# markp-gc/ipu_path_trace

Measured on AMD Instinct MI355X. Metric: Mpath-samples/sec @1104x1000, 300 spp/step, depth 8, higher is better.
Workload: dtype f16

## Files before the change

ipu_path_trace_amd/csrc/pt_nif_group.h:

```cpp
#pragma once

#include "ptmi_share_plan.h"

namespace ptd {

constexpr unsigned long long kShareEmpty = ~0ull;
constexpr uint32_t kShareMaxProbes = 32;
constexpr int kShareBlock = 256;
constexpr uint32_t kClassInFlight = 2;
static_assert(kShareBlock == (int)ptshare::kClaimBlock, "the claim tiles of ptmi_share_plan.h are for this workgroup");

__device__ __forceinline__ uint32_t share_hash(unsigned long long k) {
  k ^= k >> 33; k *= 0xff51afd7ed558ccdull;
  k ^= k >> 33; k *= 0xc4ceb9fe1a85ec53ull;
  k ^= k >> 33;
  return (uint32_t)k;
}

__device__ __forceinline__ uint32_t lane_rank(uint64_t mask) {
  return __builtin_amdgcn_mbcnt_hi((uint32_t)(mask >> 32), __builtin_amdgcn_mbcnt_lo((uint32_t)mask, 0u));
}

__device__ __forceinline__ void wave_count(bool pred, unsigned long long* ctr) {
  const uint64_t m = __ballot(pred);
// ... 403 lines not shown
  uint32_t next = s_first + ptshare::claim_wave_offset(s_appends, wave);
#pragma unroll
  for (uint32_t k = 0; k < K; ++k) {
    const uint32_t bit = 1u << k;
    const size_t q = q0 + ptshare::claim_entry(tile, threadIdx.x, k);
    const uint64_t m = __ballot((append & bit) != 0);
    if (append & bit) {
      const uint32_t i = next + lane_rank(m);
      M.c_u[i] = u[k]; M.c_v[i] = v[k];
      const uint32_t g = M.c_base + i;
      if (fresh & bit) __hip_atomic_store(M.words + slot[k], g, __ATOMIC_RELAXED, __HIP_MEMORY_SCOPE_AGENT);
      Q.owner[q] = g;
    } else if (valid & bit) {
      Q.owner[q] = ptshare::owner_is_store(word[k]) ? word[k] : ptshare::owner_class(slot[k]);
    }
    next += (uint32_t)__popcll(m);
  }
}

__global__ __launch_bounds__(kShareBlock) void class_map_claim_kernel(GroupQueue Q, ClassMap M) { class_map_claim(Q, M); }
__global__ __launch_bounds__(kShareBlock) void class_map_expand_kernel(GroupExpand E, ClassMap M) { group_expand(E, M); }
__global__ __launch_bounds__(kShareBlock) void share_raw_claim_kernel(GroupQueue Q, RawCountTable T) { group_claim(Q, T); }

__global__ __launch_bounds__(kShareBlock) void class_map_release_kernel(const float* c_u, const float* c_v, const uint32_t* c_count,
                                                                        uint32_t region, uint32_t* words) {
  const uint32_t n = c_count[blockIdx.y];
  const size_t base = (size_t)blockIdx.y * region;
  for (uint32_t i = blockIdx.x * (uint32_t)kShareBlock + threadIdx.x; i < n; i += gridDim.x * (uint32_t)kShareBlock) {
    const uint32_t slot = ptshare::class_map_index(c_u[base + i], c_v[base + i]);
    if (slot != ptshare::kClassIrregular) words[slot] = ptshare::kMapEmpty;
  }
}

__global__ __launch_bounds__(kShareBlock) void class_claim_kernel(GroupQueue Q, ClassTable T) { group_claim(Q, T); }
__global__ __launch_bounds__(kShareBlock) void class_resolve_kernel(GroupQueue Q, ClassTable T) { group_resolve(Q, T); }

__global__ __launch_bounds__(kShareBlock) void class_spread_kernel(const uint32_t* count, const uint32_t* owner, const float* class_bgr,
                                                                   float* bgr) {
  const uint32_t n = *count;
  for (uint32_t i = blockIdx.x * (uint32_t)kShareBlock + threadIdx.x; i < n; i += gridDim.x * (uint32_t)kShareBlock) {
    const float* from = class_bgr + 3 * (size_t)owner[i];
    const float b = from[0], g = from[1], r = from[2];
    float* to = bgr + 3 * (size_t)i;
    to[0] = b; to[1] = g; to[2] = r;
  }
}

}
```

ipu_path_trace_amd/csrc/pt_trace.h:

```cpp
#pragma once
#include "pt_device_math.h"
#include "pt_env_guide.h"
#include "pt_mesh.h"
#include "ptmi_trace_variant.h"

#include <utility>

namespace ptd {

enum { MAT_DIFFUSE = 0, MAT_SPECULAR = 1, MAT_REFRACTIVE = 2, MAT_EMISSIVE = 3 };
constexpr int kMaxObjects = 32;
constexpr int kBuiltinObjects = 6;
constexpr float kEps = 1e-5f;
constexpr float kInf = 3.402823466e+38f;
constexpr float kPi = 3.1415927410125732421875f;

struct SceneObject {
  float cx, cy, cz;
  float radius, r2;
  float nx, ny, nz;
  float colr, colg, colb;
  int32_t type;
  int32_t is_disc;
  float ocx, ocy, ocz;
  float c4;
  float kdisc;
  int32_t same_centre;
// ... 24 lines not shown
constexpr int kHitObjectBits = 5;
static_assert((1 << kHitObjectBits) == kMaxObjects, "5 bits of object in a packed hit");

struct TraceParams {
  SceneObject obj[kMaxObjects];
  uint32_t n_objects;
  float width_f, height_f;
  uint32_t width, height;
  float tx, ty;
  float aa_scale;
  float stop_prob;
  float rr_factor;
  float ri;
  float azimuth;
  uint32_t seed_lo, seed_hi;
  uint32_t sample_base;
  uint32_t max_path_length, roulette_depth;
  int32_t aa_type, samples_half;
  uint32_t n_items, total_paths;
  uint32_t n_waves;
  uint32_t region_cap;
  int32_t env_const;
  float env_r, env_g, env_b;
  const uint32_t* pix;
  float* q_u; float* q_v; float* q_tr; float* q_tg; float* q_tb; uint32_t* q_path;
  uint32_t* region_count;
  uint8_t* plen;
  float* rad_r; float* rad_g; float* rad_b;
  uint4* survivors;
  float4* states;
  size_t state_stride;
  uint32_t div_magic, div_shift;
  unsigned long long* diag;
  unsigned long long* emitted;
  int32_t cam_pose;
  float cam_r[3], cam_u[3], cam_f[3];
  float lens_a, lens_f;
  GuideParams guide;
  LightParams lights;
  PolyEdges poly[kMaxObjects];
  const ptmesh::Node* mesh_nodes;
  const ptmesh::F4* mesh_tris;
  const uint32_t* mesh_orig;
  const ptmesh::F4* mesh_normals;
};
static_assert(sizeof(TraceParams) <= 4096, "the scene travels in the kernel arguments: 4 KiB at most");
// ... 557 lines not shown
  if (s.depth >= P.max_path_length) {
    length = s.depth;
    return STEP_DEAD;
  }
  return STEP_CONTINUE;
}

__device__ __forceinline__ void dir_to_uv(Vec3 d, float azimuth, float& u, float& v) {
  float theta = dm_acos(d.y);
  float phi = dm_atan2(d.z, d.x) + azimuth;
  const float twoPi = 2.f * kPi;
  const float invPi = 1.f / kPi;
  const float inv2Pi = 1.f / twoPi;
  if (phi < 0.f) phi += twoPi;
  else if (phi > twoPi) phi -= twoPi;
  u = theta * invPi;
  v = phi * inv2Pi;
}

constexpr int kTraceBlock = 256;
constexpr uint32_t kRefillThreshold = 16;

__device__ __forceinline__ uint32_t emit_emitted(const TraceParams& P, bool emitted, Vec3 rad, uint32_t idx) {
  if (emitted) { P.rad_r[idx] = rad.x; P.rad_g[idx] = rad.y; P.rad_b[idx] = rad.z; }
  return (uint32_t)__popcll(__ballot(emitted));
}

template <int CAM = CAM_BUILTIN>
__device__ __forceinline__ void emit_escaped(const TraceParams& P, bool escaped, const PathState& st, uint32_t idx, uint32_t lane,
                                             uint32_t region_base, uint32_t* wg_count) {
  if (P.env_const) {
    if (escaped) {
      P.rad_r[idx] = P.env_r * st.T.x;
      P.rad_g[idx] = P.env_g * st.T.y;
      P.rad_b[idx] = P.env_b * st.T.z;
    }
    return;
  }
  const uint64_t esc_mask = __ballot(escaped);
  if (!esc_mask) return;
  uint32_t base = 0;
  if (lane == (uint32_t)__ffsll((long long)esc_mask) - 1u) base = atomicAdd(wg_count, (uint32_t)__popcll(esc_mask));
  base = __shfl(base, __ffsll((long long)esc_mask) - 1, 64);
  if (escaped) {
    const uint32_t rank = __builtin_amdgcn_mbcnt_hi((uint32_t)(esc_mask >> 32), __builtin_amdgcn_mbcnt_lo((uint32_t)esc_mask, 0u));
    const uint32_t q = region_base + base + rank;
    float u, v;
    Vec3 d = st.d;
    if constexpr (CAM != CAM_BUILTIN) { if (CAM == CAM_POSE || P.cam_pose) d = to_world(P, d); }
    dir_to_uv(d, P.azimuth, u, v);
    P.q_u[q] = u; P.q_v[q] = v;
    P.q_tr[q] = st.T.x; P.q_tg[q] = st.T.y; P.q_tb[q] = st.T.z;
    P.q_path[q] = idx;
  }
}

__device__ __forceinline__ uint32_t pack_half2(float a, float b) {
  union { _Float16 h[2]; uint32_t u; } c;
  c.h[0] = (_Float16)a; c.h[1] = (_Float16)b;
  return c.u;
}

#ifdef PTMI_DIAG_BUILD
}
#include "diag/pt_trace_r3fn.h"
#include "diag/pt_trace_rounds.h"
namespace ptd {
#endif

constexpr int kTraceOpt = 3;
template <uint32_t REFILL, int OPT = kTraceOpt, int CAM = CAM_BUILTIN, bool GUIDE = false, bool LIGHTS = false, bool POLY = false,
          bool PLAMPS = false, bool MESH = false, bool SMOOTH = false, bool TEX = false>
__device__ __forceinline__ void trace_body(const TraceParams& P, [[maybe_unused]] const TexParams* X = nullptr) {
  constexpr bool MAGIC = (OPT & 1) != 0, PRIMARY = (OPT & 2) != 0, SCENE_C = (OPT & 128) != 0, PIPE = (OPT & 256) != 0;
  __shared__ uint32_t wg_count;
  __shared__ uint32_t wg_front, wg_back;
// ... 332 lines not shown
```

ipu_path_trace_amd/csrc/ptmi.hip:

```cpp
#include <hip/hip_runtime.h>
#include <rccl/rccl.h>

#include <dlfcn.h>
#include <limits.h>

#include <algorithm>
#include <array>
#include <atomic>
#include <chrono>
#include <cmath>
#include <cfloat>
#include <cstdio>
#include <cstdlib>
#include <condition_variable>
#include <cstring>
#include <deque>
#include <functional>
#include <memory>
#include <mutex>
#include <string>
#include <thread>
#include <utility>
#include <vector>

// ... 513 lines not shown
        if (h->env_const) return PT_OK;
        ptd::NifParams N = h->nif;
        if (mode.classes)
          bind_dense_queue(N, h->group.d_class_u + b.class_base, h->group.d_class_v + b.class_base, h->group.d_class_count + b.index,
                           b.store_cap, h->group.d_class_bgr + 3 * (size_t)b.class_base);
        else if (mode.grouped()) bind_store_queue(h, N, b.index, b.store_base, b.store_cap);
        else bind_path_queue(N, B, b.g.blocks, b.g.region_cap);
#ifdef PTMI_DIAG_BUILD
        if (h->diag_fault_batch >= 0 && (uint32_t)h->diag_fault_batch == b.index)
          return fail(h, PT_ERR_HIP, "injected fault: NIF launch of batch " + std::to_string(b.index));
#endif
        if (int rc = h->env_map ? launch_envmap(h, N) : launch_nif(h, N, h->n_cus)) return rc;
        B.last_paths = b.total; B.last_regions = b.g.blocks; B.last_region_cap = b.g.region_cap;
        B.share_batch = mode.grouped() ? (int32_t)b.index : -1; B.share_base = b.store_base; B.share_region_cap = b.store_cap;
        h->stats.nif_launches += 1;
        return PT_OK;
      }, &done)) return rc;
  if (mode.classes && !mode.fused())
    if (int rc = stage_class_spread(h, ev, b, &done)) return rc;
  PT_HIP(hipStreamWaitEvent(h->acc_stream, done, 0));
  return PT_OK;
}

static int stage_accumulate(pt_handle h, StepEvents& ev, const Batch& b) {
  const pt_context::BatchBuffers& B = *b.B;
  const uint32_t n = h->n_items;
  if (int rc = ev.timed(h->acc_stream, pt_context::kSpanAccumulate, [&]() -> int {
        if (n % 4u == 0)
          hipLaunchKernelGGL(ptd::accumulate4_kernel, dim3((n / 4u + 255) / 256), dim3(256), 0, h->acc_stream, n, b.iters, B.plen,
                             B.rad_r, B.rad_g, B.rad_b, h->acc, h->d_counters);
        else
          hipLaunchKernelGGL(ptd::accumulate_kernel, dim3((n + 255) / 256), dim3(256), 0, h->acc_stream, n, b.iters, B.plen, B.rad_r,
                             B.rad_g, B.rad_b, h->acc, h->d_counters);
        PT_HIP(hipGetLastError());
        return PT_OK;
      })) return rc;
  PT_HIP(hipEventRecord(B.accumulated, h->acc_stream));
  h->stats.trace_launches += 1;
  h->stats.accumulate_launches += 1;
  return PT_OK;
}

static int enqueue_path_trace(pt_handle h) {
  const uint32_t n = h->n_items;
  if (int rc = ensure_meshes(h)) return rc;
  forget_replay_state(h);
  PT_HIP(hipMemsetAsync(h->d_counters, 0, 4 * sizeof(unsigned long long), h->stream));
  ptd::TraceParams P;
  fill_trace_params(h, P);
  P.n_items = n;
  StepEvents ev{h};
  hipEvent_t e_begin = nullptr, e_acc = nullptr, e_end = nullptr, e_class_cleared = nullptr;
  size_t e_acc_i = 0;
  if (int rc = ev.record(h->stream, e_begin, h->e_begin_i)) return rc;
  PT_HIP(hipStreamWaitEvent(h->trace_stream, e_begin, 0));
  const std::vector<uint32_t> deal = ptplan::batch_iterations(h->samples_per_step, h->iters_per_batch, h->first_batch_iters, h->env_const);
  const uint32_t batches = (uint32_t)deal.size();
  const int32_t share = h->group.share_mode_set ? h->group.share_mode : auto_share_mode(h, batches);
  StepMode mode{h->env_const ? 0 : share, !h->env_const && h->group.memo_slots != 0};
  h->group.share_mode_last = mode.share;
  h->group.memo_ran = mode.memo;
  if (mode.grouped()) {
    if (int rc = prepare_group_store(h, mode, batches)) return rc;
    if (int rc = prepare_class_level(h, ev, batches, mode, e_class_cleared)) return rc;
  }
  h->group.class_ran = mode.classes;
  if (mode.memo)
    if (int rc = ev.timed(h->trace_stream, pt_context::kSpanMemo, [&]() { return enqueue_memo_prologue(h); })) return rc;

  const bool handoff = mode.kind() == ptshare::StepKind::kStep;
  hipEvent_t e_clean = nullptr;
  uint32_t store_cap = 0, first_iter = 0;
  for (uint32_t i = 0; i < batches; first_iter += deal[i], ++i) {
    const uint32_t slot = ptplan::ring_slot(i, h->ring_depth);
    Batch b{i, first_iter, deal[i], deal[i] * n, trace_grid(deal[i] * n, h->trace_blocks), &h->bb[slot], 0u, 0u, slot};
    b.store_base = mode.grouped() ? ptplan::store_region(i, h->ring_depth, mode.step_scope()) * (uint32_t)h->queue_cap : 0u;
    b.store_cap = b.g.blocks * b.g.region_cap;
    b.class_base = mode.classes ? i * (uint32_t)h->queue_cap : 0u;
    store_cap = std::max(store_cap, b.store_cap);
    if (mode.mapped && ptplan::ring_predecessor(i, h->ring_depth) != ptplan::kNoBatch)
      PT_HIP(hipStreamWaitEvent(h->trace_stream, b.B->raw_read, 0));
    if (int rc = stage_trace(h, ev, P, b)) return rc;
    if (mode.grouped())
      if (int rc = stage_group(h, ev, mode, b, e_class_cleared)) return rc;
    if (int rc = stage_nif(h, ev, mode, b)) return rc;
    if (handoff && i + 1 == batches && !mode.mapped)
      if (int rc = enqueue_table_handoff(h, ev, e_clean, h->trace_stream)) return rc;
    if (mode.grouped())
      if (int rc = stage_expand(h, ev, mode, b)) return rc;
    if (int rc = stage_accumulate(h, ev, b)) return rc;
    if (mode.mapped)
      if (int rc = stage_raw_pairs(h, ev, b)) return rc;
    if (handoff && i + 1 == batches && mode.mapped)
      if (int rc = enqueue_table_handoff(h, ev, e_clean, h->acc_stream)) return rc;
  }
  if (e_clean) PT_HIP(hipStreamWaitEvent(h->stream, e_clean, 0));

  if (mode.mapped)
    if (int rc = stage_map_release(h, ev, store_cap, batches)) return rc;
  if (int rc = ev.record(h->acc_stream, e_acc, e_acc_i)) return rc;
  PT_HIP(hipStreamWaitEvent(h->stream, e_acc, 0));
  if (mode.memo)
    if (int rc = stage_memo_publish(h, ev, store_cap, batches)) return rc;
  PT_HIP(hipMemcpyAsync(h->h_counters, h->d_counters, 4 * sizeof(unsigned long long), hipMemcpyDeviceToHost, h->stream));
  if (mode.grouped()) {
    PT_HIP(hipMemcpyAsync(h->group.h_share_count, h->group.d_share_count, (size_t)batches * 4, hipMemcpyDeviceToHost, h->stream));
    PT_HIP(hipMemcpyAsync(h->group.h_share_over, h->group.d_share_over, 8, hipMemcpyDeviceToHost, h->stream));
  }
  if (mode.classes) {
    PT_HIP(hipMemcpyAsync(h->group.h_class_count, h->group.d_class_count, (size_t)batches * 4, hipMemcpyDeviceToHost, h->stream));
    PT_HIP(hipMemcpyAsync(h->group.h_class_over, h->group.d_class_over, 8, hipMemcpyDeviceToHost, h->stream));
  }
  if (mode.memo) PT_HIP(hipMemcpyAsync(h->group.h_memo_ctr, h->group.d_memo_ctr, ptd::kMemoCounters * 8, hipMemcpyDeviceToHost, h->stream));
// ... 13 lines not shown
    else if (s.kind == pt_context::kSpanShare) h->group.share_ms += ms;
    else if (s.kind == pt_context::kSpanClass) h->group.class_ms += ms;
    else h->group.memo_ms += ms;
  }
  float total_ms = 0.f;
  PT_HIP(hipEventElapsedTime(&total_ms, h->events[h->e_begin_i], h->events[h->e_end_i]));
  h->stats.total_ms = total_ms;
  return PT_OK;
}

extern "C" {

int pt_path_trace(pt_handle h) {
  if (!h) return PT_ERR_INVALID_ARGUMENT;
  if (!h->settings_valid) return fail(h, PT_ERR_NOT_READY, "pt_set_render_settings has not been called");
  if (!h->env_const && !h->env_map && !h->nif_valid)
    return fail(h, PT_ERR_NOT_READY, "no environment: call pt_upload_nif, pt_set_env_map or pt_set_constant_env");
  PT_HIP(hipSetDevice(h->cfg.device));
  memset(&h->stats, 0, sizeof(h->stats));
  h->group.share_mode_last = 0; h->group.share_evals = 0; h->group.share_overflowed = 0; h->group.share_ms = 0;
  h->group.memo_ran = false; h->group.memo_served = 0; h->group.memo_inserted = 0; h->group.memo_ms = 0;
  h->group.class_ran = false; h->group.class_rows = 0; h->group.class_alone = 0; h->group.class_ms = 0;
  h->group.class_map_ran = false;
  h->spans_pending = false;
  h->stats.nif_flops_per_sample = (h->env_const || h->env_map) ? 0 : h->nif_flops;
  h->stats.first_sample = h->sample_cursor;
  const uint32_t n = h->n_items;
  if (n == 0) return PT_OK;

  h->spans.clear();
  const int rc = enqueue_path_trace(h);
  hipError_t s0 = hipStreamSynchronize(h->stream), s1 = hipSuccess, s2 = hipSuccess, s3 = hipSuccess;
  if (rc || s0 != hipSuccess) {
    for (hipStream_t cs : h->chunk_stream) { const hipError_t e = hipStreamSynchronize(cs); if (e != hipSuccess) s3 = e; }
    s1 = hipStreamSynchronize(h->trace_stream);
    s2 = hipStreamSynchronize(h->acc_stream);
    (void)hipStreamSynchronize(h->stream);
  }
  const bool failed = rc || s0 != hipSuccess || s1 != hipSuccess || s2 != hipSuccess || s3 != hipSuccess;
  if (failed) memo_new_generation(h);
  h->group.share_clean_slots = ptshare::mark_after_step(h->group.share_clean_slots,
      StepMode{h->group.share_mode_last, h->group.memo_ran}.kind(), h->group.share_slots, !failed);
  h->group.class_map_clean = ptshare::map_mark_after_step(h->group.class_map_clean, h->group.class_map_ran, !failed);
  if (rc) return rc;
  for (hipError_t e : {s0, s1, s2, s3})
    if (e != hipSuccess) return fail(h, PT_ERR_HIP, std::string("path_trace: ") + hipGetErrorString(e));
// ... 752 lines not shown
```

ipu_path_trace_amd/csrc/ptmi_context.h:

```cpp
#pragma once

using ptplan::TraceGrid;
using ptplan::trace_grid;
using ptplan::item_divider;

namespace {

thread_local std::string g_create_error;

inline uint32_t f2u(float f) { uint32_t u; memcpy(&u, &f, 4); return u; }
inline float u2f(uint32_t u) { float f; memcpy(&f, &u, 4); return f; }

uint16_t host_f2h(float f) {
  uint32_t x = f2u(f), sign = (x >> 16) & 0x8000u, ax = x & 0x7fffffffu;
  if (ax >= 0x7f800000u) return (uint16_t)(sign | 0x7c00u | ((ax > 0x7f800000u) ? 0x200u : 0u));
  if (ax >= 0x477ff000u) return (uint16_t)(sign | 0x7c00u);
  if (ax < 0x33000001u) return (uint16_t)sign;
  int e = (int)(ax >> 23) - 127;
  uint32_t m = (ax & 0x7fffffu) | 0x800000u, shift, hexp;
  if (e < -14) { shift = (uint32_t)(13 + (-14 - e)); hexp = 0; } else { shift = 13; hexp = (uint32_t)(e + 15); }
  uint32_t q = m >> shift, rem = m & ((1u << shift) - 1u), halfway = 1u << (shift - 1);
  if (rem > halfway || (rem == halfway && (q & 1u))) q += 1u;
  uint32_t h = hexp == 0 ? q : ((hexp - 1u) << 10) + q;
  return (uint16_t)(sign | h);
// ... 285 lines not shown

    DevBuf<unsigned long long> d_class_keys;
    DevBuf<uint32_t> d_class_vals;
    uint32_t class_slots = 0;
    uint32_t class_diag_slots = 0;
    DevBuf<uint32_t> d_class_owner;
    DevBuf<float> d_class_u, d_class_v, d_class_bgr;
    size_t class_regions = 0;
    DevBuf<uint32_t> d_class_count;
    DevBuf<unsigned long long> d_class_over;
    PinnedBuf<uint32_t> h_class_count;
    PinnedBuf<unsigned long long> h_class_over;
    size_t class_count_cap = 0;
    bool class_failed = false;
    bool class_ran = false;
    uint64_t class_rows = 0, class_alone = 0;
    double class_ms = 0;
    DevBuf<uint32_t> d_class_map;
    DevBuf<unsigned long long> d_class_tail_keys;
    uint32_t class_tail_slots = 0;
    bool class_map_clean = false;
    bool class_map_failed = false;
    bool class_map_ran = false;

    DevBuf<ptd::MemoSlot> d_memo;
    uint32_t memo_slots = 0;
    DevBuf<ptd::MemoSlot> d_memo_list;
    DevBuf<uint32_t> d_memo_slot;
    size_t memo_slot_regions = 0;
    DevBuf<unsigned long long> d_memo_ctr;
    PinnedBuf<unsigned long long> h_memo_ctr;
    bool memo_clear = false;
    uint32_t memo_step = 0;
    bool memo_ran = false;
    uint64_t memo_occupied = 0, memo_served = 0, memo_inserted = 0, memo_generation = 0, memo_retains = 0;
    double memo_ms = 0;
  } group;

  pt_stats stats{};
  std::vector<hipEvent_t> events;
  enum SpanKind { kSpanNone = -1, kSpanTrace, kSpanNif, kSpanAccumulate, kSpanShare, kSpanMemo, kSpanClass };
  struct StageSpan { size_t a, b; int kind; };
  std::vector<StageSpan> spans;
  size_t e_begin_i = 0, e_end_i = 0;
  bool spans_pending = false;

// ... 308 lines not shown
```

ipu_path_trace_amd/csrc/ptmi_nif_group.h:

```cpp
#pragma once

static int resolve_stage_times(pt_handle h);


static uint64_t free_device_bytes() {
  size_t free_b = 0, total_b = 0;
  return hipMemGetInfo(&free_b, &total_b) == hipSuccess ? (uint64_t)free_b : ptshare::kFreeUnknown;
}

static uint32_t share_table_slots(pt_handle h, uint64_t entries, uint64_t free_b) {
  if (h->group.share_diag_slots) return h->group.share_diag_slots;
  return ptshare::worst_case_slots(entries, free_b);
}

static int ensure_share_counts(pt_handle h, size_t batches) {
  if (batches <= h->group.share_count_cap) return PT_OK;
  h->group.share_count_cap = 0;
  PT_HIP(dev_alloc(h->group.d_share_count, batches));
  PT_HIP(dev_alloc(h->group.h_share_count, batches));
  h->group.share_count_cap = batches;
  return PT_OK;
}

static int ensure_share_store(pt_handle h, size_t regions) {
// ... 113 lines not shown
  } else if (2 * h->group.memo_occupied > h->group.memo_slots) {
    const uint32_t list_cap = std::max<uint32_t>(1, h->group.memo_slots / 2);
    const uint32_t grid = std::min<uint32_t>(ptd::kMemoGrid, (h->group.memo_slots + ptd::kShareBlock - 1) / ptd::kShareBlock);
    hipLaunchKernelGGL(ptd::memo_compact_kernel, dim3(grid), dim3(ptd::kShareBlock), 0, s, h->group.d_memo, h->group.memo_slots, last,
                       h->group.d_memo_list, list_cap, h->group.d_memo_ctr);
    PT_HIP(hipGetLastError());
    PT_HIP(hipMemsetAsync(h->group.d_memo, 0xff, table_bytes, s));
    PT_HIP(hipMemsetAsync(h->group.d_memo_ctr + ptd::kMemoOccupied, 0, 8, s));
    const uint32_t rgrid = std::min<uint32_t>(ptd::kMemoGrid, (list_cap + ptd::kShareBlock - 1) / ptd::kShareBlock);
    hipLaunchKernelGGL(ptd::memo_reinsert_kernel, dim3(rgrid), dim3(ptd::kShareBlock), 0, s, h->group.d_memo, h->group.memo_slots - 1u,
                       h->group.d_memo_list, list_cap, h->group.d_memo_ctr);
    PT_HIP(hipGetLastError());
    h->group.memo_retains += 1;
  }
  return PT_OK;
}

struct StepMode {
  int32_t share;
  bool memo;
  bool classes = false;
  bool fused() const { return classes && !memo && share == PT_NIF_SHARE_STEP; }
  bool mapped = false;
  bool grouped() const { return share || memo; }
  bool step_scope() const { return memo || share == PT_NIF_SHARE_STEP; }
  ptshare::StepKind kind() const {
    return memo ? ptshare::StepKind::kMemo : share == PT_NIF_SHARE_STEP ? ptshare::StepKind::kStep
           : share == PT_NIF_SHARE_BATCH ? ptshare::StepKind::kBatch : ptshare::StepKind::kOff;
  }
};

static int32_t auto_share_mode(pt_handle h, size_t batches) {
  if (h->env_const || h->env_map || h->group.memo_slots || h->group.share_auto_failed) return PT_NIF_SHARE_OFF;
  const uint64_t free_b = free_device_bytes();
  const uint64_t slots = share_table_slots(h, batches * (uint64_t)h->queue_cap, free_b);
  ptshare::Held held;
  held.table_slots = h->group.d_share_keys ? (h->group.share_diag_slots ? slots : h->group.share_slots) : 0;
  held.store_regions = h->group.share_regions;
  for (const auto& o : h->group.d_share_owner) held.owner_maps += o ? 1 : 0;
  if (!ptshare::auto_fits(slots, batches, h->queue_cap, held, free_b, pt_context::kBatchSets)) return PT_NIF_SHARE_OFF;
  if (ensure_group_buffers(h, false, true, batches) == PT_OK && alloc_group_buffers(h) == PT_OK) return PT_NIF_SHARE_STEP;
  (void)hipGetLastError();
  free_share_buffers(h);
  h->group.share_auto_failed = true;
  h->error.clear();
  return PT_NIF_SHARE_OFF;
// ... 214 lines not shown
          else hipLaunchKernelGGL(ptd::share_claim_kernel, tiles, block, 0, h->trace_stream, Q, share_table(h));
        }
        PT_HIP(hipGetLastError());
        return PT_OK;
      })) return rc;
  return resolve_on_nif_stream(mode) ? PT_OK : stage_resolve(h, ev, mode, b, h->trace_stream);
}

static int stage_expand(pt_handle h, StepEvents& ev, const StepMode& mode, const Batch& b) {
  return ev.timed(h->acc_stream, mode.memo ? pt_context::kSpanMemo : pt_context::kSpanShare, [&]() -> int {
    const pt_context::BatchBuffers& B = *b.B;
    ptd::GroupExpand X;
    X.region_count = B.region_count;
    X.region_cap = b.g.region_cap;
    X.owner = h->group.d_share_owner[b.set()];
    X.bgr = mode.fused() ? h->group.d_class_bgr : h->group.d_share_bgr;
    X.q_tr = B.q_tr; X.q_tg = B.q_tg; X.q_tb = B.q_tb; X.q_path = B.q_path;
    X.rad_r = B.rad_r; X.rad_g = B.rad_g; X.rad_b = B.rad_b;
    if (mode.memo) hipLaunchKernelGGL(ptd::memo_expand_kernel, b.group_grid(), dim3(ptd::kShareBlock), 0, h->acc_stream, X, memo_table(h));
    else if (mode.mapped) hipLaunchKernelGGL(ptd::class_map_expand_kernel, b.group_grid(), dim3(ptd::kShareBlock), 0, h->acc_stream, X, class_map(h, b));
    else if (mode.fused()) hipLaunchKernelGGL(ptd::share_class_expand_kernel, b.group_grid(), dim3(ptd::kShareBlock), 0, h->acc_stream, X, share_class_table(h, b));
    else hipLaunchKernelGGL(ptd::share_expand_kernel, b.group_grid(), dim3(ptd::kShareBlock), 0, h->acc_stream, X, share_table(h));
    PT_HIP(hipGetLastError());
    return PT_OK;
  });
}

static int stage_raw_pairs(pt_handle h, StepEvents& ev, const Batch& b) {
  if (int rc = ev.timed(h->acc_stream, pt_context::kSpanShare, [&]() -> int {
        hipLaunchKernelGGL(ptd::share_raw_claim_kernel, b.claim_grid(), dim3(ptd::kShareBlock), 0, h->acc_stream, group_queue(h, b),
                           ptd::RawCountTable{share_table(h)});
        PT_HIP(hipGetLastError());
        return PT_OK;
      })) return rc;
  PT_HIP(hipEventRecord(b.B->raw_read, h->acc_stream));
  return PT_OK;
}

static int stage_map_release(pt_handle h, StepEvents& ev, uint32_t store_cap, uint32_t batches) {
  return ev.timed(h->acc_stream, pt_context::kSpanShare, [&]() -> int {
    const dim3 grid(std::min<uint32_t>(ptd::kMemoGrid, (store_cap + ptd::kShareBlock - 1u) / ptd::kShareBlock), batches);
    hipLaunchKernelGGL(ptd::class_map_release_kernel, grid, dim3(ptd::kShareBlock), 0, h->acc_stream, h->group.d_class_u, h->group.d_class_v,
                       h->group.d_class_count, (uint32_t)h->queue_cap, h->group.d_class_map);
    PT_HIP(hipGetLastError());
    PT_HIP(hipMemsetAsync(h->group.d_class_map + ptshare::kClassMapWords, 0xff, (size_t)h->group.class_tail_slots * 4, h->acc_stream));
    PT_HIP(hipMemsetAsync(h->group.d_class_tail_keys, 0xff, (size_t)h->group.class_tail_slots * 8, h->acc_stream));
    return PT_OK;
  });
}

static int stage_memo_publish(pt_handle h, StepEvents& ev, uint32_t store_cap, uint32_t batches) {
  return ev.timed(h->stream, pt_context::kSpanMemo, [&]() -> int {
    const dim3 grid(std::min<uint32_t>(ptd::kMemoGrid, (store_cap + ptd::kShareBlock - 1u) / ptd::kShareBlock), batches);
    hipLaunchKernelGGL(ptd::memo_publish_kernel, grid, dim3(ptd::kShareBlock), 0, h->stream, h->group.d_memo, h->group.d_memo_slot,
                       h->group.d_share_bgr, h->group.d_share_count, (uint32_t)h->queue_cap, h->group.memo_step);
    PT_HIP(hipGetLastError());
    return PT_OK;
  });
}

extern "C" {

int pt_set_nif_sharing(pt_handle h, int32_t mode) {
  if (!h) return PT_ERR_INVALID_ARGUMENT;
  if (mode != PT_NIF_SHARE_OFF && mode != PT_NIF_SHARE_BATCH && mode != PT_NIF_SHARE_STEP)
    return fail(h, PT_ERR_INVALID_ARGUMENT, "pt_set_nif_sharing: mode must be PT_NIF_SHARE_OFF, _BATCH or _STEP");
  if (mode != PT_NIF_SHARE_OFF) {
    PT_HIP(hipSetDevice(h->cfg.device));
    if (int rc = alloc_share_buffers(h)) { h->group.share_mode = PT_NIF_SHARE_OFF; h->group.share_mode_set = true; return rc; }
// ... 158 lines not shown
  PT_HIP(hipMemcpyAsync(owner, own, n * 4, hipMemcpyDeviceToHost, s));
  PT_HIP(hipMemcpyAsync(d_u, du, n * 4, hipMemcpyDeviceToHost, s));
  PT_HIP(hipMemcpyAsync(d_v, dv, n * 4, hipMemcpyDeviceToHost, s));
  PT_HIP(hipMemcpyAsync(d_count, len, 4, hipMemcpyDeviceToHost, s));
  PT_HIP(hipMemcpyAsync(overflowed, over, 8, hipMemcpyDeviceToHost, s));
  if (memo == 1 && memo_counters) PT_HIP(hipMemcpyAsync(memo_counters, ctr, ptd::kMemoCounters * 8, hipMemcpyDeviceToHost, s));
  if (table_keys) {
    if (memo == 1) PT_HIP(hipMemcpy2DAsync(table_keys, 8, slots, sizeof(ptd::MemoSlot), 8, table_slots, hipMemcpyDeviceToHost, s));
    else PT_HIP(hipMemcpyAsync(table_keys, keys, (size_t)table_slots * 8, hipMemcpyDeviceToHost, s));
  }
  PT_HIP(hipStreamSynchronize(s));
  return PT_OK;
}

int pt_diag_set_nif_class_capacity(pt_handle h, uint32_t slots) {
  if (!h || slots > ptshare::kClassMaxSlots) return PT_ERR_INVALID_ARGUMENT;
  uint32_t p = slots ? 2 : 0;
  while (p < slots) p <<= 1;
  h->group.class_diag_slots = p;
  h->group.class_failed = false;
  return PT_OK;
}

int pt_diag_class_claim(pt_handle h, const float* u, const float* v, uint32_t n, uint32_t table_slots, uint32_t* owner, float* c_u,
                        float* c_v, uint32_t* c_count, uint64_t* alone) {
  if (!h || !u || !v || !owner || !c_u || !c_v || !c_count || !alone) return PT_ERR_INVALID_ARGUMENT;
  if (n == 0 || n >= ptshare::kMaxStoreEntries || table_slots < 2 || table_slots > ptshare::kClassMaxSlots || (table_slots & (table_slots - 1u)))
    return fail(h, PT_ERR_INVALID_ARGUMENT, "pt_diag_class_claim: sizes out of range");
  PT_HIP(hipSetDevice(h->cfg.device));
  hipStream_t s = h->stream;
  DevBuf<float> q_u, q_v, du, dv;
  DevBuf<uint32_t> count, own, len, vals;
  DevBuf<unsigned long long> over, keys;
  PT_HIP(dev_alloc(q_u, n)); PT_HIP(dev_alloc(q_v, n)); PT_HIP(dev_alloc(du, n)); PT_HIP(dev_alloc(dv, n));
  PT_HIP(dev_alloc(count, 1)); PT_HIP(dev_alloc(own, n)); PT_HIP(dev_alloc(len, 1)); PT_HIP(dev_alloc(over, 1));
  PT_HIP(dev_alloc(keys, table_slots)); PT_HIP(dev_alloc(vals, table_slots));
  PT_HIP(hipMemcpyAsync(q_u, u, (size_t)n * 4, hipMemcpyHostToDevice, s));
  PT_HIP(hipMemcpyAsync(q_v, v, (size_t)n * 4, hipMemcpyHostToDevice, s));
  PT_HIP(hipMemcpyAsync(count, &n, 4, hipMemcpyHostToDevice, s));
  PT_HIP(hipMemsetAsync(own, 0xff, (size_t)n * 4, s));
  PT_HIP(hipMemsetAsync(over, 0, 8, s));
  PT_HIP(hipMemsetAsync(len, 0, 4, s));
  PT_HIP(hipMemsetAsync(keys, 0xff, (size_t)table_slots * 8, s));
  ptd::GroupQueue Q;
  Q.q_u = q_u; Q.q_v = q_v; Q.region_count = count; Q.region_cap = n; Q.owner = own;
  Q.d_u = du; Q.d_v = dv; Q.d_count = len; Q.base = 0; Q.overflowed = over;
// ... 100 lines not shown
  PT_HIP(hipSetDevice(h->cfg.device));
  hipStream_t s = h->stream;
  DevBuf<float> q_u, q_v, cu, cv;
  DevBuf<uint32_t> counts, own, row, len, words;
  DevBuf<unsigned long long> over, tail_keys;
  PT_HIP(dev_alloc(q_u, n)); PT_HIP(dev_alloc(q_v, n)); PT_HIP(dev_alloc(cu, 2 * n)); PT_HIP(dev_alloc(cv, 2 * n));
  PT_HIP(dev_alloc(counts, n_regions)); PT_HIP(dev_alloc(own, n)); PT_HIP(dev_alloc(row, n)); PT_HIP(dev_alloc(len, 1)); PT_HIP(dev_alloc(over, 3));
  PT_HIP(dev_alloc(words, n_words)); PT_HIP(dev_alloc(tail_keys, tail_slots));
  PT_HIP(hipMemcpyAsync(q_u, u, n * 4, hipMemcpyHostToDevice, s));
  PT_HIP(hipMemcpyAsync(q_v, v, n * 4, hipMemcpyHostToDevice, s));
  PT_HIP(hipMemcpyAsync(counts, region_count, (size_t)n_regions * 4, hipMemcpyHostToDevice, s));
  PT_HIP(hipMemsetAsync(over, 0, 24, s));
  PT_HIP(hipMemsetAsync(len, 0, 4, s));
  PT_HIP(hipMemsetAsync(words, 0xff, n_words * 4, s));
  PT_HIP(hipMemsetAsync(tail_keys, 0xff, (size_t)tail_slots * 8, s));
  ptd::GroupQueue Q;
  Q.q_u = q_u; Q.q_v = q_v; Q.region_count = counts; Q.region_cap = region_cap; Q.owner = own;
  Q.d_u = nullptr; Q.d_v = nullptr; Q.d_count = nullptr; Q.base = 0; Q.overflowed = nullptr;
  const ptd::ClassMap M{words, tail_keys, tail_slots - 1u, cu, cv, len, 0u, over};
  const dim3 grid((region_cap + ptd::kShareBlock - 1u) / ptd::kShareBlock, n_regions), tiles(ptshare::claim_tiles(region_cap), n_regions);
  const dim3 block(ptd::kShareBlock), count_grid(ptd::kMemoGrid);
  auto release = [&]() -> int {
    hipLaunchKernelGGL(ptd::class_map_release_kernel, dim3(std::min<uint32_t>(ptd::kMemoGrid, (uint32_t)((2 * n + ptd::kShareBlock - 1u) / ptd::kShareBlock)), 1),
                       block, 0, s, cu, cv, len, 0u, words);
    PT_HIP(hipGetLastError());
    PT_HIP(hipMemsetAsync(words + ptshare::kClassMapWords, 0xff, (size_t)tail_slots * 4, s));
    PT_HIP(hipMemsetAsync(tail_keys, 0xff, (size_t)tail_slots * 8, s));
    return PT_OK;
  };
  for (uint32_t launch = 0; launch < launches; ++launch) {
    if (launch && release_between) {
      if (int rc = release()) return rc;
      PT_HIP(hipMemsetAsync(len, 0, 4, s));
      PT_HIP(hipMemsetAsync(over, 0, 8, s));
    }
    PT_HIP(hipMemsetAsync(own, 0xff, n * 4, s));
    hipLaunchKernelGGL(ptd::class_map_claim_kernel, tiles, block, 0, s, Q, M);
    PT_HIP(hipGetLastError());
  }
  hipLaunchKernelGGL(ptd::diag_map_hop_kernel, grid, block, 0, s, counts, region_cap, own, words, row);
  PT_HIP(hipGetLastError());
  hipLaunchKernelGGL(ptd::diag_map_count_kernel, count_grid, block, 0, s, words, (uint32_t)n_words, over + 1);
  PT_HIP(hipGetLastError());
  if (int rc = release()) return rc;
  hipLaunchKernelGGL(ptd::diag_map_count_kernel, count_grid, block, 0, s, words, (uint32_t)n_words, over + 2);
  PT_HIP(hipGetLastError());
  uint32_t h_len = 0;
  unsigned long long h_over[3] = {0, 0, 0};
  PT_HIP(hipMemcpyAsync(owner, own, n * 4, hipMemcpyDeviceToHost, s));
  PT_HIP(hipMemcpyAsync(rows, row, n * 4, hipMemcpyDeviceToHost, s));
// ... 13 lines not shown
```

ipu_path_trace_amd/csrc/ptmi_share_plan.h:

```cpp
#pragma once

#include <cstdint>

namespace ptshare {

constexpr uint32_t kOwnerTagged = 0x80000000u;
constexpr uint32_t kOwnerPending = 0xc0000000u;
constexpr uint32_t kOwnerSlotBits = 0x3fffffffu;
constexpr uint32_t owner_served(uint32_t slot) { return kOwnerTagged | slot; }
constexpr uint32_t owner_pending(uint32_t slot) { return kOwnerPending | slot; }
constexpr bool owner_is_store(uint32_t o) { return !(o & kOwnerTagged); }
constexpr bool owner_is_pending(uint32_t o) { return (o & kOwnerPending) == kOwnerPending; }
constexpr bool owner_is_served(uint32_t o) { return (o & kOwnerPending) == kOwnerTagged; }
constexpr uint32_t owner_slot(uint32_t o) { return o & kOwnerSlotBits; }

constexpr uint32_t owner_class(uint32_t class_slot) { return kOwnerTagged | class_slot; }
constexpr bool owner_is_class(uint32_t o) { return (o & kOwnerPending) == kOwnerTagged; }
constexpr uint32_t kNoWriteBack = ~0u;
template <class RawVals, class ClassVals>
constexpr uint32_t resolve_two_hops(uint32_t o, const RawVals& raw_vals, const ClassVals& class_vals, uint32_t* write_back = nullptr) {
  if (write_back) *write_back = kNoWriteBack;
  if (owner_is_pending(o)) {
    const uint32_t s = owner_slot(o);
    o = raw_vals[s];
// ... 85 lines not shown
}
constexpr uint32_t class_coord(float coord) { return class_x((coord - 1.0f) * 2.0f); }
constexpr uint64_t class_key(float u, float v) { return ((uint64_t)class_coord(u) << 32) | (uint64_t)class_coord(v); }

constexpr uint32_t kClassAxis = ((kClassMaxMag - kClassMinMag) >> 13) + 1u;
constexpr uint32_t kClassMapWords = kClassAxis * kClassAxis;
constexpr uint32_t kClassIrregular = ~0u;
constexpr uint32_t kClassTailSlots = 1u << 16;
constexpr uint32_t kClassTailMaxSlots = 1u << 20;
static_assert((uint64_t)kClassMapWords + kClassTailMaxSlots - 1 <= kOwnerSlotBits, "a class slot fits an owner word");
constexpr uint32_t kMapEmpty = 0xffffffffu;
constexpr uint32_t kMapClaimed = 0xfffffffeu;
constexpr uint32_t class_axis_index(uint32_t c) {
  const uint32_t mag = c & 0x7fffffffu;
  return (c >> 31) && !(c & 0x1fffu) && mag >= kClassMinMag && mag <= kClassMaxMag ? (mag - kClassMinMag) >> 13 : kClassIrregular;
}
constexpr uint32_t class_map_index(float u, float v) {
  const uint32_t iu = class_axis_index(class_coord(u)), iv = class_axis_index(class_coord(v));
  return iu == kClassIrregular || iv == kClassIrregular ? kClassIrregular : iu * kClassAxis + iv;
}
constexpr uint64_t class_map_bytes(uint32_t tail_slots) { return ((uint64_t)kClassMapWords + tail_slots) * 4 + (uint64_t)tail_slots * 8; }
constexpr bool map_clear_skippable(bool mark) { return mark; }
constexpr bool map_mark_after_step(bool mark, bool used, bool ok) { return used ? ok : mark; }
inline bool class_map_fits(bool held, uint32_t tail_slots, uint64_t free_bytes, uint64_t also = 0) {
  if (held) return true;
  if (free_bytes == kFreeUnknown) return false;
  return class_map_bytes(tail_slots) + also <= free_bytes / kAutoMemoryDivisor;
}

constexpr uint64_t kClassSpace = 16385ull * 16385ull;
constexpr uint64_t kClassMaxSlots = 1ull << 29;
inline uint32_t class_slots(uint64_t entries, uint64_t free_bytes) {
  uint64_t want = kMinSlots;
  while (want < 2ull * entries && want < kClassMaxSlots) want <<= 1;
  if (free_bytes != kFreeUnknown)
    while (want > kMinSlots && want * kSlotBytes > free_bytes / kTableMemoryDivisor) want >>= 1;
  return (uint32_t)want;
}
struct ClassHeld {
  uint64_t table_slots = 0, store_regions = 0, owner_maps = 0;
};
inline uint64_t class_bytes(uint64_t table_slots, uint64_t batches, uint64_t queue_cap, const ClassHeld& held) {
  uint64_t need = 0;
  if (table_slots > held.table_slots) need += table_slots * kSlotBytes;
  if (batches > held.store_regions) need += batches * queue_cap * kStoreEntryBytes;
  if (!held.owner_maps) need += queue_cap * kOwnerEntryBytes;
// ... 13 lines not shown
```

ipu_path_trace_amd/ptmi.py:

```python
import ctypes as C
import os

import numpy as np

from .build import library_path

TRACE_DTYPE = np.dtype([("u", "<u2"), ("v", "<u2"), ("r", "<f4"), ("g", "<f4"), ("b", "<f4"),
                        ("sampleCount", "<u2"), ("pathLength", "<u2")], align=True)
assert TRACE_DTYPE.itemsize == 20

PATH_DTYPE = np.dtype([("length", "<u4"), ("escaped", "<u4"), ("dir", "<f4", 3), ("uv", "<f4", 2),
                       ("throughput", "<f4", 3), ("cam", "<f4", 2)])
assert PATH_DTYPE.itemsize == 48

SCENE_DTYPE = np.dtype([("shape", "<i4"), ("material", "<i4"), ("centre", "<f4", 3), ("radius", "<f4"),
                        ("normal", "<f4", 3), ("colour", "<f4", 3)])
assert SCENE_DTYPE.itemsize == 48
SCENE_EX_DTYPE = np.dtype(SCENE_DTYPE.descr + [("vertex", "<f4", (3, 3))])
assert SCENE_EX_DTYPE.itemsize == 84
MAX_SCENE_OBJECTS = 32
SHAPE_SPHERE, SHAPE_DISC = 0, 1
SHAPE_TRIANGLE, SHAPE_PARALLELOGRAM = 2, 3
SHAPE_MESH = 4
MAX_MESH_TRIANGLES = 1 << 22
# ... 655 lines not shown
    L.pt_denoise_default_params.argtypes = [C.POINTER(DenoiseParams)]
    L.pt_denoise.argtypes = [C.c_void_p, C.POINTER(DenoiseParams), C.c_int32, C.c_void_p, C.c_void_p]
    L.pt_nif_train_default_params.argtypes = [C.POINTER(NifTrainParams)]
    L.pt_nif_train_begin.argtypes = [C.c_void_p, C.POINTER(NifTrainParams)]
    L.pt_nif_train_layer_shapes.argtypes = [C.c_void_p, C.POINTER(Layer), C.c_uint32]
    L.pt_nif_train_steps.argtypes = [C.c_void_p, C.c_uint32, C.POINTER(C.c_float)]
    L.pt_nif_train_get_weights.argtypes = [C.c_void_p, C.POINTER(Layer), C.c_uint32]
    L.pt_nif_train_set_weights.argtypes = [C.c_void_p, C.POINTER(Layer), C.c_uint32]
    L.pt_nif_train_get_encode_params.argtypes = [C.c_void_p, C.POINTER(C.c_float), C.POINTER(C.c_float)]
    L.pt_nif_train_export.argtypes = [C.c_void_p, C.POINTER(Layer), C.c_uint32]
    L.pt_nif_train_install.argtypes = [C.c_void_p]
    L.pt_nif_train_end.argtypes = [C.c_void_p]
    L.pt_nif_train_batch.argtypes = [C.c_void_p, C.c_uint64, C.c_void_p, C.c_void_p, C.c_void_p]
    L.pt_nif_train_default_precision.argtypes = [C.POINTER(NifTrainPrecision)]
    L.pt_nif_train_set_precision.argtypes = [C.c_void_p, C.POINTER(NifTrainPrecision)]
    L.pt_nif_train_get_precision_state.argtypes = [C.c_void_p, C.POINTER(NifTrainPrecisionState)]
    L.pt_nif_train_gradients.argtypes = [C.c_void_p, C.c_void_p, C.c_void_p, C.c_void_p, C.c_uint32, C.POINTER(C.c_float),
                                         C.POINTER(Layer), C.c_uint32]
    if diag:
        L.pt_diag_set_nif_share_capacity.argtypes = [C.c_void_p, C.c_uint32]
        L.pt_diag_set_nif_memo_slots.argtypes = [C.c_void_p, C.c_uint32]
        L.pt_diag_claim_resolve.argtypes = [C.c_void_p, C.c_int32, C.c_uint32] + [C.c_void_p] * 3 + [C.c_uint32] * 3 + [C.c_void_p] * 7
        L.pt_diag_set_nif_class_capacity.argtypes = [C.c_void_p, C.c_uint32]
        L.pt_diag_class_claim.argtypes = [C.c_void_p, C.c_void_p, C.c_void_p, C.c_uint32, C.c_uint32] + [C.c_void_p] * 5
        L.pt_diag_share_class_claim.argtypes = [C.c_void_p] * 4 + [C.c_uint32] * 4 + [C.c_void_p] * 6
        L.pt_diag_class_map_claim.argtypes = [C.c_void_p] * 4 + [C.c_uint32] * 4 + [C.c_int32] + [C.c_void_p] * 5
        L.pt_diag_inject_fault.argtypes = [C.c_void_p, C.c_int32]
        L.pt_diag_stamps.argtypes = [C.c_void_p, C.c_void_p]
        L.pt_diag_nif_clock.argtypes = [C.c_void_p, C.c_void_p]
        L.pt_diag_comm_self_exchange.argtypes = [C.c_void_p, C.c_size_t, C.POINTER(C.c_int)]
        L.pt_diag_denoise_bench.argtypes = [C.c_void_p, C.c_int32, C.c_uint32, C.c_uint32, C.POINTER(C.c_double)]
    _libs[diag] = L
    return L


def degrees_to_radians_f32(deg):
    return float(np.float32(deg) * np.float32(np.pi / 180.0))


def rotation_to_radians_f32(deg):
    return float(np.float32((np.float32(deg) / np.float32(360.0)) * (2.0 * np.pi)))


class Renderer:

    def __init__(self, width, height, max_work_items=None, max_path_length=10, roulette_depth=3, stop_prob=0.3,
# ... 733 lines not shown
```

Before: 10200.

## Fold mapped expand pass into accumulate via inverse queue-slot index

When class mapping is active and sizes fit 32-bit addressing, the trace kernel writes an inverse path-to-queue-slot index instead of queue-to-path. A new accumulate kernel then gathers owner colours through the class map and multiplies them by throughput directly, so the separate expand kernel launch and its intermediate radiance writes are skipped. The release kernel also clears the tail slots and keys itself, replacing two memset calls. The cost is a gather-heavy accumulate with indirect loads, plus an extra store of the no-slot marker for emitted paths.

```diff
diff --git a/ipu_path_trace_amd/csrc/pt_nif_group.h b/ipu_path_trace_amd/csrc/pt_nif_group.h
--- a/ipu_path_trace_amd/csrc/pt_nif_group.h
+++ b/ipu_path_trace_amd/csrc/pt_nif_group.h
@@ -449,13 +449,115 @@
 __global__ __launch_bounds__(kShareBlock) void class_map_expand_kernel(GroupExpand E, ClassMap M) { group_expand(E, M); }
 __global__ __launch_bounds__(kShareBlock) void share_raw_claim_kernel(GroupQueue Q, RawCountTable T) { group_claim(Q, T); }
 
+struct MappedGather {
+  const uint32_t* slot;
+  const uint32_t* owner;
+  const uint32_t* words;
+  const float* bgr;
+  const float* q_tr; const float* q_tg; const float* q_tb;
+  const float* rad_r; const float* rad_g; const float* rad_b;
+};
+struct MappedStage {
+  uint32_t pl;
+  uint32_t q[4];
+  uint32_t o[4];
+  __device__ __forceinline__ bool has(uint32_t c) const { return q[c] != ptshare::kNoQueueSlot; }
+  __device__ __forceinline__ uint32_t slot(uint32_t c) const { return has(c) ? q[c] : 0u; }
+};
+template <class T>
+__device__ __forceinline__ T at32(const T* base, uint32_t index) {
+  static_assert(sizeof(T) == 4 || sizeof(T) == 8, "4-byte elements, one or two of them");
+  return *reinterpret_cast<const T*>(reinterpret_cast<const char*>(base) + (uint32_t)(index * 4u));
+}
+__device__ __forceinline__ void mapped_load_slots(const MappedGather& G, const uint8_t* plen, uint32_t n, uint32_t iters, uint32_t i,
+                                                  uint32_t k, MappedStage& s) {
+  uint32_t w[2];
+  uint2 v[2];
+#pragma unroll
+  for (uint32_t j = 0; j < 2; ++j) {
+    const uint32_t p = (k + j < iters ? k + j : iters - 1u) * n + i;
+    w[j] = *reinterpret_cast<const uint16_t*>(plen + p);
+    v[j] = at32(reinterpret_cast<const uint2*>(G.slot), p);
+    if (k + j >= iters) w[j] = 0u;
+  }
+  s.pl = w[0] | (w[1] << 16);
+  const uint32_t q[4] = {v[0].x, v[0].y, v[1].x, v[1].y};
+#pragma unroll
+  for (uint32_t c = 0; c < 4; ++c) s.q[c] = ((s.pl >> (8u * c + 7u)) & 1u) ? q[c] : ptshare::kNoQueueSlot;
+}
+__device__ __forceinline__ void mapped_load_owners(const MappedGather& G, MappedStage& s) {
+#pragma unroll
+  for (uint32_t c = 0; c < 4; ++c) s.o[c] = at32(G.owner, s.slot(c));
+}
+__global__ __launch_bounds__(256) void accumulate_mapped_kernel(uint32_t n, uint32_t iters, const uint8_t* plen, MappedGather G, Accum A,
+                                                                 unsigned long long* counters) {
+  const uint32_t i = 2u * (blockIdx.x * blockDim.x + threadIdx.x);
+  uint32_t segs = 0, esc = 0;
+  if (i < n) {
+    float2 r = *reinterpret_cast<const float2*>(A.r + i), g = *reinterpret_cast<const float2*>(A.g + i),
+           b = *reinterpret_cast<const float2*>(A.b + i);
+    uint32_t len[2] = {0, 0};
+    MappedStage sa, sb, sc;
+    mapped_load_slots(G, plen, n, iters, i, 0u, sa);
+    mapped_load_slots(G, plen, n, iters, i, 2u, sb);
+    mapped_load_owners(G, sa);
+    float* const rc[2] = {&r.x, &r.y};
+    float* const gc[2] = {&g.x, &g.y};
+    float* const bc[2] = {&b.x, &b.y};
+    for (uint32_t k = 0; k < iters; k += 2u) {
+      mapped_load_slots(G, plen, n, iters, i, k + 4u, sc);
+      mapped_load_owners(G, sb);
+      float x[4][3], t[4][3];
+#pragma unroll
+      for (uint32_t c = 0; c < 4; ++c) {
+        uint32_t o = sa.has(c) ? sa.o[c] : 0u;
+        if (!ptshare::owner_is_store(o)) o = G.words[ptshare::owner_slot(o)];
+        const float* held = G.bgr + 3 * (size_t)o;
+        x[c][0] = held[0]; x[c][1] = held[1]; x[c][2] = held[2];
+        t[c][0] = at32(G.q_tr, sa.slot(c)); t[c][1] = at32(G.q_tg, sa.slot(c)); t[c][2] = at32(G.q_tb, sa.slot(c));
+      }
+      const uint32_t w = sa.pl;
+      len[0] += (w & 0x7fu) + ((w >> 16) & 0x7fu); len[1] += ((w >> 8) & 0x7fu) + ((w >> 24) & 0x7fu);
+#pragma unroll
+      for (uint32_t c = 0; c < 4; ++c) {
+        if (!((w >> (8u * c + 7u)) & 1u)) continue;
+        float vr = x[c][2] * t[c][0], vg = x[c][1] * t[c][1], vb = x[c][0] * t[c][2];
+        if (!sa.has(c)) {
+          const uint32_t p = (k + (c >> 1)) * n + i + (c & 1u);
+          vr = G.rad_r[p]; vg = G.rad_g[p]; vb = G.rad_b[p];
+        }
+        *rc[c & 1u] += vr; *gc[c & 1u] += vg; *bc[c & 1u] += vb;
+      }
+      esc += (uint32_t)__popc(w & 0x80808080u);
+      sa = sb; sb = sc;
+    }
+    *reinterpret_cast<float2*>(A.r + i) = r;
+    *reinterpret_cast<float2*>(A.g + i) = g;
+    *reinterpret_cast<float2*>(A.b + i) = b;
+    uint2 cnt = *reinterpret_cast<const uint2*>(A.count + i), ln = *reinterpret_cast<const uint2*>(A.length + i);
+    cnt.x += iters; cnt.y += iters;
+    ln.x += len[0]; ln.y += len[1];
+    *reinterpret_cast<uint2*>(A.count + i) = cnt;
+    *reinterpret_cast<uint2*>(A.length + i) = ln;
+    segs = len[0] + len[1];
+  }
+  accumulate_counters(segs, esc, counters);
+}
+
 __global__ __launch_bounds__(kShareBlock) void class_map_release_kernel(const float* c_u, const float* c_v, const uint32_t* c_count,
-                                                                        uint32_t region, uint32_t* words) {
+                                                                        uint32_t region, uint32_t* words, unsigned long long* tail_keys,
+                                                                        uint32_t tail_slots) {
   const uint32_t n = c_count[blockIdx.y];
   const size_t base = (size_t)blockIdx.y * region;
   for (uint32_t i = blockIdx.x * (uint32_t)kShareBlock + threadIdx.x; i < n; i += gridDim.x * (uint32_t)kShareBlock) {
     const uint32_t slot = ptshare::class_map_index(c_u[base + i], c_v[base + i]);
     if (slot != ptshare::kClassIrregular) words[slot] = ptshare::kMapEmpty;
+  }
+  if (blockIdx.y == 0) {
+    for (uint32_t i = blockIdx.x * (uint32_t)kShareBlock + threadIdx.x; i < tail_slots; i += gridDim.x * (uint32_t)kShareBlock) {
+      words[ptshare::kClassMapWords + i] = ptshare::kMapEmpty;
+      tail_keys[i] = kShareEmpty;
+    }
   }
 }
 
diff --git a/ipu_path_trace_amd/csrc/pt_trace.h b/ipu_path_trace_amd/csrc/pt_trace.h
--- a/ipu_path_trace_amd/csrc/pt_trace.h
+++ b/ipu_path_trace_amd/csrc/pt_trace.h
@@ -3,6 +3,7 @@
 #include "pt_env_guide.h"
 #include "pt_mesh.h"
 #include "ptmi_trace_variant.h"
+#include "ptmi_share_plan.h"
 
 #include <utility>
 
@@ -73,6 +74,7 @@
   uint32_t region_cap;
   int32_t env_const;
   float env_r, env_g, env_b;
+  uint32_t q_inverse;
   const uint32_t* pix;
   float* q_u; float* q_v; float* q_tr; float* q_tg; float* q_tb; uint32_t* q_path;
   uint32_t* region_count;
@@ -676,7 +678,10 @@
 constexpr uint32_t kRefillThreshold = 16;
 
 __device__ __forceinline__ uint32_t emit_emitted(const TraceParams& P, bool emitted, Vec3 rad, uint32_t idx) {
-  if (emitted) { P.rad_r[idx] = rad.x; P.rad_g[idx] = rad.y; P.rad_b[idx] = rad.z; }
+  if (emitted) {
+    P.rad_r[idx] = rad.x; P.rad_g[idx] = rad.y; P.rad_b[idx] = rad.z;
+    if (P.q_inverse) P.q_path[idx] = ptshare::kNoQueueSlot;
+  }
   return (uint32_t)__popcll(__ballot(emitted));
 }
 
@@ -705,7 +710,7 @@
     dir_to_uv(d, P.azimuth, u, v);
     P.q_u[q] = u; P.q_v[q] = v;
     P.q_tr[q] = st.T.x; P.q_tg[q] = st.T.y; P.q_tb[q] = st.T.z;
-    P.q_path[q] = idx;
+    P.q_path[P.q_inverse ? idx : q] = P.q_inverse ? q : idx;
   }
 }
 
diff --git a/ipu_path_trace_amd/csrc/ptmi.hip b/ipu_path_trace_amd/csrc/ptmi.hip
--- a/ipu_path_trace_amd/csrc/ptmi.hip
+++ b/ipu_path_trace_amd/csrc/ptmi.hip
@@ -559,11 +559,18 @@
   return PT_OK;
 }
 
-static int stage_accumulate(pt_handle h, StepEvents& ev, const Batch& b) {
+static int stage_accumulate(pt_handle h, StepEvents& ev, const StepMode& mode, const Batch& b) {
   const pt_context::BatchBuffers& B = *b.B;
   const uint32_t n = h->n_items;
   if (int rc = ev.timed(h->acc_stream, pt_context::kSpanAccumulate, [&]() -> int {
-        if (n % 4u == 0)
+        if (mode.expand_in_accumulate) {
+          if (b.total > h->queue_cap || h->queue_cap >= ptshare::kMaxSlotsAt32 || (uint64_t)b.g.blocks * b.g.region_cap > h->queue_cap)
+            return fail(h, PT_ERR_INVALID_ARGUMENT, "accumulate: a batch's paths or queue slots exceed what the expanding pass addresses");
+          const ptd::MappedGather G{B.q_path, h->group.d_share_owner[b.set()], h->group.d_class_map, h->group.d_class_bgr,
+                                    B.q_tr, B.q_tg, B.q_tb, B.rad_r, B.rad_g, B.rad_b};
+          hipLaunchKernelGGL(ptd::accumulate_mapped_kernel, dim3((n / 2u + 255) / 256), dim3(256), 0, h->acc_stream, n, b.iters, B.plen,
+                             G, h->acc, h->d_counters);
+        } else if (n % 4u == 0)
           hipLaunchKernelGGL(ptd::accumulate4_kernel, dim3((n / 4u + 255) / 256), dim3(256), 0, h->acc_stream, n, b.iters, B.plen,
                              B.rad_r, B.rad_g, B.rad_b, h->acc, h->d_counters);
         else
@@ -602,6 +609,11 @@
     if (int rc = prepare_class_level(h, ev, batches, mode, e_class_cleared)) return rc;
   }
   h->group.class_ran = mode.classes;
+  mode.expand_in_accumulate = ptshare::expands_in_accumulate(mode.mapped, n, h->queue_cap);
+#ifdef PTMI_DIAG_BUILD
+  if (getenv("PTMI_EXPAND_PASS")) mode.expand_in_accumulate = false;
+#endif
+  P.q_inverse = mode.expand_in_accumulate ? 1u : 0u;
   if (mode.memo)
     if (int rc = ev.timed(h->trace_stream, pt_context::kSpanMemo, [&]() { return enqueue_memo_prologue(h); })) return rc;
 
@@ -623,9 +635,9 @@
     if (int rc = stage_nif(h, ev, mode, b)) return rc;
     if (handoff && i + 1 == batches && !mode.mapped)
       if (int rc = enqueue_table_handoff(h, ev, e_clean, h->trace_stream)) return rc;
-    if (mode.grouped())
+    if (mode.grouped() && !mode.expand_in_accumulate)
       if (int rc = stage_expand(h, ev, mode, b)) return rc;
-    if (int rc = stage_accumulate(h, ev, b)) return rc;
+    if (int rc = stage_accumulate(h, ev, mode, b)) return rc;
     if (mode.mapped)
       if (int rc = stage_raw_pairs(h, ev, b)) return rc;
     if (handoff && i + 1 == batches && mode.mapped)
@@ -685,6 +697,7 @@
   h->group.memo_ran = false; h->group.memo_served = 0; h->group.memo_inserted = 0; h->group.memo_ms = 0;
   h->group.class_ran = false; h->group.class_rows = 0; h->group.class_alone = 0; h->group.class_ms = 0;
   h->group.class_map_ran = false;
+  h->group.expand_launches = 0;
   h->spans_pending = false;
   h->stats.nif_flops_per_sample = (h->env_const || h->env_map) ? 0 : h->nif_flops;
   h->stats.first_sample = h->sample_cursor;
diff --git a/ipu_path_trace_amd/csrc/ptmi_context.h b/ipu_path_trace_amd/csrc/ptmi_context.h
--- a/ipu_path_trace_amd/csrc/ptmi_context.h
+++ b/ipu_path_trace_amd/csrc/ptmi_context.h
@@ -331,6 +331,7 @@
     bool class_map_clean = false;
     bool class_map_failed = false;
     bool class_map_ran = false;
+    uint32_t expand_launches = 0;
 
     DevBuf<ptd::MemoSlot> d_memo;
     uint32_t memo_slots = 0;
diff --git a/ipu_path_trace_amd/csrc/ptmi_nif_group.h b/ipu_path_trace_amd/csrc/ptmi_nif_group.h
--- a/ipu_path_trace_amd/csrc/ptmi_nif_group.h
+++ b/ipu_path_trace_amd/csrc/ptmi_nif_group.h
@@ -159,6 +159,7 @@
   bool classes = false;
   bool fused() const { return classes && !memo && share == PT_NIF_SHARE_STEP; }
   bool mapped = false;
+  bool expand_in_accumulate = false;
   bool grouped() const { return share || memo; }
   bool step_scope() const { return memo || share == PT_NIF_SHARE_STEP; }
   ptshare::StepKind kind() const {
@@ -419,6 +420,7 @@
     else if (mode.fused()) hipLaunchKernelGGL(ptd::share_class_expand_kernel, b.group_grid(), dim3(ptd::kShareBlock), 0, h->acc_stream, X, share_class_table(h, b));
     else hipLaunchKernelGGL(ptd::share_expand_kernel, b.group_grid(), dim3(ptd::kShareBlock), 0, h->acc_stream, X, share_table(h));
     PT_HIP(hipGetLastError());
+    h->group.expand_launches += 1;
     return PT_OK;
   });
 }
@@ -438,10 +440,8 @@
   return ev.timed(h->acc_stream, pt_context::kSpanShare, [&]() -> int {
     const dim3 grid(std::min<uint32_t>(ptd::kMemoGrid, (store_cap + ptd::kShareBlock - 1u) / ptd::kShareBlock), batches);
     hipLaunchKernelGGL(ptd::class_map_release_kernel, grid, dim3(ptd::kShareBlock), 0, h->acc_stream, h->group.d_class_u, h->group.d_class_v,
-                       h->group.d_class_count, (uint32_t)h->queue_cap, h->group.d_class_map);
-    PT_HIP(hipGetLastError());
-    PT_HIP(hipMemsetAsync(h->group.d_class_map + ptshare::kClassMapWords, 0xff, (size_t)h->group.class_tail_slots * 4, h->acc_stream));
-    PT_HIP(hipMemsetAsync(h->group.d_class_tail_keys, 0xff, (size_t)h->group.class_tail_slots * 8, h->acc_stream));
+                       h->group.d_class_count, (uint32_t)h->queue_cap, h->group.d_class_map, h->group.d_class_tail_keys, h->group.class_tail_slots);
+    PT_HIP(hipGetLastError());
     return PT_OK;
   });
 }
@@ -646,6 +646,12 @@
   return PT_OK;
 }
 
+int pt_diag_expand_launches(pt_handle h, uint32_t* launches) {
+  if (!h || !launches) return PT_ERR_INVALID_ARGUMENT;
+  *launches = h->group.expand_launches;
+  return PT_OK;
+}
+
 int pt_diag_class_claim(pt_handle h, const float* u, const float* v, uint32_t n, uint32_t table_slots, uint32_t* owner, float* c_u,
                         float* c_v, uint32_t* c_count, uint64_t* alone) {
   if (!h || !u || !v || !owner || !c_u || !c_v || !c_count || !alone) return PT_ERR_INVALID_ARGUMENT;
@@ -792,10 +798,8 @@
   const dim3 block(ptd::kShareBlock), count_grid(ptd::kMemoGrid);
   auto release = [&]() -> int {
     hipLaunchKernelGGL(ptd::class_map_release_kernel, dim3(std::min<uint32_t>(ptd::kMemoGrid, (uint32_t)((2 * n + ptd::kShareBlock - 1u) / ptd::kShareBlock)), 1),
-                       block, 0, s, cu, cv, len, 0u, words);
-    PT_HIP(hipGetLastError());
-    PT_HIP(hipMemsetAsync(words + ptshare::kClassMapWords, 0xff, (size_t)tail_slots * 4, s));
-    PT_HIP(hipMemsetAsync(tail_keys, 0xff, (size_t)tail_slots * 8, s));
+                       block, 0, s, cu, cv, len, 0u, words, tail_keys, tail_slots);
+    PT_HIP(hipGetLastError());
     return PT_OK;
   };
   for (uint32_t launch = 0; launch < launches; ++launch) {
diff --git a/ipu_path_trace_amd/csrc/ptmi_share_plan.h b/ipu_path_trace_amd/csrc/ptmi_share_plan.h
--- a/ipu_path_trace_amd/csrc/ptmi_share_plan.h
+++ b/ipu_path_trace_amd/csrc/ptmi_share_plan.h
@@ -131,6 +131,17 @@
 constexpr uint64_t class_map_bytes(uint32_t tail_slots) { return ((uint64_t)kClassMapWords + tail_slots) * 4 + (uint64_t)tail_slots * 8; }
 constexpr bool map_clear_skippable(bool mark) { return mark; }
 constexpr bool map_mark_after_step(bool mark, bool used, bool ok) { return used ? ok : mark; }
+constexpr uint64_t kMaxSlotsAt32 = 1ull << 30;
+constexpr bool expands_in_accumulate(bool mapped, uint32_t work_items, uint64_t queue_cap) {
+  return mapped && work_items % 4u == 0 && queue_cap < kMaxSlotsAt32;
+}
+constexpr uint32_t kNoQueueSlot = 0xffffffffu;
+static_assert(kNoQueueSlot >= kMaxStoreEntries, "the marker is no queue slot");
+template <class Words>
+constexpr uint32_t mapped_row(uint32_t owner_word, const Words& words) {
+  return owner_is_store(owner_word) ? owner_word : words[owner_slot(owner_word)];
+}
+
 inline bool class_map_fits(bool held, uint32_t tail_slots, uint64_t free_bytes, uint64_t also = 0) {
   if (held) return true;
   if (free_bytes == kFreeUnknown) return false;
diff --git a/ipu_path_trace_amd/ptmi.py b/ipu_path_trace_amd/ptmi.py
--- a/ipu_path_trace_amd/ptmi.py
+++ b/ipu_path_trace_amd/ptmi.py
@@ -701,6 +701,7 @@
         L.pt_diag_set_nif_memo_slots.argtypes = [C.c_void_p, C.c_uint32]
         L.pt_diag_claim_resolve.argtypes = [C.c_void_p, C.c_int32, C.c_uint32] + [C.c_void_p] * 3 + [C.c_uint32] * 3 + [C.c_void_p] * 7
         L.pt_diag_set_nif_class_capacity.argtypes = [C.c_void_p, C.c_uint32]
+        L.pt_diag_expand_launches.argtypes = [C.c_void_p, C.POINTER(C.c_uint32)]
         L.pt_diag_class_claim.argtypes = [C.c_void_p, C.c_void_p, C.c_void_p, C.c_uint32, C.c_uint32] + [C.c_void_p] * 5
         L.pt_diag_share_class_claim.argtypes = [C.c_void_p] * 4 + [C.c_uint32] * 4 + [C.c_void_p] * 6
         L.pt_diag_class_map_claim.argtypes = [C.c_void_p] * 4 + [C.c_uint32] * 4 + [C.c_int32] + [C.c_void_p] * 5
```

After: 10620 (median of 6 runs). +4.2%, better.
